# yupbank/tensorframes

Measured on AMD Instinct MI355X. Metric: rows/sec map_blocks MatMul on 10M-row DF at 1/2/4/8 MI355X, higher is better.
Workload: dtype fp32; 1 GPU; model=map_blocks relu(matmul(x[?,512], W[512,512])) float32, global_batch=10000000, seq_len=512, parallelism=dp1, partitions=4, rows=10000000

## Files before the change

### csrc/kernels/conv_wino.hip

```cpp
#include <algorithm>
#include <atomic>
#include <cstdlib>
#include <cstring>

#include "gemm_f32_core.h"

namespace tfa {
namespace k {

namespace {

typedef float f32x4 __attribute__((ext_vector_type(4)));
typedef float f32x16 __attribute__((ext_vector_type(16)));

struct WinoGeom {
  int H, W, C, OH, OW, pt, pl, TH, TW, OCP, KT;
  int64_t ntiles;
  int64_t img_floats;
  int64_t u_bytes;
  int dbg;
  int axis, D0, D1;
  FastDivU32 fD0, fD1;
  int KTC;
  FastDivU32 fKTC;
// ... 129 lines not shown
    }
    filt(1);
    filt(2);
#pragma unroll
    for (int m = 0; m < MT; ++m) {
      const f32x4 t3v = tr(inp(ra, 3, m), inp(rb, 3, m));
      av[3][m] = t1v[m] - t3v;
    }
    filt(3);
  };

  f32x16 acc[4][2];
  auto mfma_cols = [&](int j0, int j1, const f32x4 (&a)[4][MT], const f32x4 (&b)[4][NT]) __attribute__((always_inline)) {
#pragma unroll
    for (int j = j0; j < j1; ++j)
#pragma unroll
      for (int s = 0; s < 4; ++s)
#pragma unroll
        for (int m = 0; m < MT; ++m)
#pragma unroll
          for (int nh = 0; nh < NT; ++nh)
            acc[j][m * NT + nh] = __builtin_amdgcn_mfma_f32_32x32x2f32(a[j][m][s], b[j][nh][s], acc[j][m * NT + nh], 0, 0, 0);
  };
  f32x4 pa[4][MT], pb[4][NT];
  float* E = reinterpret_cast<float*>(smem + STAGE);

  int item = f32core::xcd_remap(blockIdx.x, G);
  if (item >= nwork) return;
  Item cur;
  setup(item, true, cur);
  issue(cur, 0);
  for (bool first = true;; first = false) {
#pragma unroll
    for (int j = 0; j < 4; ++j)
#pragma unroll
      for (int k2 = 0; k2 < 2; ++k2) acc[j][k2] = (f32x16){};
    for (int kt = 0; kt < KT; ++kt) {
      if (kt == 0 && !first) wwait_vm<NST>();
      else wwait_vm<0>();
      __builtin_amdgcn_s_barrier();
      if (kt + 1 < KT) issue(cur, kt + 1);
      if (kt > 0) mfma_cols(3, 4, pa, pb);
      read(kt);
      mfma_cols(0, 3, av, bv);
#pragma unroll
      for (int m = 0; m < MT; ++m) pa[3][m] = av[3][m];
#pragma unroll
      for (int nh = 0; nh < NT; ++nh) pb[3][nh] = bv[3][nh];
    }
    mfma_cols(3, 4, pa, pb);
    const int cq = lane % LPT, trr = lane / LPT;
    const int64_t col = cur.n0 + 4 * cq;
    const bool colok = col < g.N;
    float* cbase;
    int64_t cld;
    int cact;
    f32core::out_col(g, static_cast<float*>(g.C), colok ? col : 0, cbase, cld, cact);
    const float* bias = static_cast<const float*>(g.bias);
    const float4 bvv = (bias && colok) ? *reinterpret_cast<const float4*>(bias + col) : make_float4(0.f, 0.f, 0.f, 0.f);
    __syncthreads();
    const int next = item + G;
    const bool live = next < nwork;
    Item nx;
    setup(next, live, nx);
    issue(nx, 0);
    float4 pmax[NPASS];
#pragma unroll
    for (int px = 0; px < 2; ++px) {
#pragma unroll
      for (int m = 0; m < MT; ++m)
#pragma unroll
        for (int nh = 0; nh < NT; ++nh)
#pragma unroll
          for (int r = 0; r < 16; ++r) {
            const int k2 = m * NT + nh;
            const float mv = px == 0 ? (acc[0][k2][r] + acc[1][k2][r]) + acc[2][k2][r]
                                     : (acc[1][k2][r] - acc[2][k2][r]) - acc[3][k2][r];
            const int tile = (tp * MT + m) * TWV + (r & 3) + 8 * (r >> 2) + 4 * h;
            E[(xr * T + tile) * EP + 32 * nh + r32] = mv;
          }
      asm volatile("s_waitcnt lgkmcnt(0)" ::: "memory");
      __builtin_amdgcn_s_barrier();
#pragma unroll
      for (int ps = 0; ps < NPASS; ++ps) {
        const int tile = wave * (T / 8) + ps * TPP + trr;
        const int64_t t = cur.t0 + tile;
        const bool tl = t < q.ntiles;
        const uint32_t tc = tl ? (uint32_t)t : 0u, qa = fdiv(tc, q.fTW), tx = tc - qa * (uint32_t)q.TW;
        const uint32_t n = fdiv(qa, q.fTH), ty = qa - n * (uint32_t)q.TH;
        f32x4 e[4];
#pragma unroll
        for (int w = 0; w < 4; ++w) e[w] = *reinterpret_cast<const f32x4*>(&E[(w * T + tile) * EP + 4 * cq]);
        const f32x4 y0 = (e[0] + e[1]) + e[2];
        const f32x4 y1 = (e[1] - e[2]) - e[3];
        const int ow = 2 * (int)tx + px;
        float4 ov[2];
#pragma unroll
        for (int py = 0; py < 2; ++py) {
          const f32x4 v = py ? y1 : y0;
          ov[py].x = act3(v[0] + bvv.x, cact);
          ov[py].y = act3(v[1] + bvv.y, cact);
          ov[py].z = act3(v[2] + bvv.z, cact);
          ov[py].w = act3(v[3] + bvv.w, cact);
        }
        if constexpr (POOL) {
          const float4 m = make_float4(fmaxf(ov[0].x, ov[1].x), fmaxf(ov[0].y, ov[1].y), fmaxf(ov[0].z, ov[1].z),
                                       fmaxf(ov[0].w, ov[1].w));
          if (px == 0) {
            pmax[ps] = m;
          } else {
// ... 126 lines not shown
    av[7] = (d[7] - d[1]) + c21 * (d[3] - d[5]);
    const f32x4 e1 = (d[2] + d[6]) - c17 * d[4], o1 = (d[1] + d[5]) - c17 * d[3];
    av[1] = e1 + o1;
    av[2] = e1 - o1;
    const f32x4 e3 = (0.25f * d[2] + d[6]) - c5q * d[4], o3 = (0.5f * d[1] + 2.f * d[5]) - c5h * d[3];
    av[3] = e3 + o3;
    av[4] = e3 - o3;
    const f32x4 e5 = (4.f * d[2] + d[6]) - c5 * d[4], o5 = (2.f * d[1] + 0.5f * d[5]) - c5h * d[3];
    av[5] = e5 + o5;
    av[6] = e5 - o5;
  };

  f32x16 acc[8];
  auto mfma_pts = [&](int x0, int x1, const f32x4 (&a)[8], const f32x4 (&b)[8]) __attribute__((always_inline)) {
#pragma unroll
    for (int xi = x0; xi < x1; ++xi)
#pragma unroll
      for (int st = 0; st < 4; ++st) acc[xi] = __builtin_amdgcn_mfma_f32_32x32x2f32(a[xi][st], b[xi][st], acc[xi], 0, 0, 0);
  };
  f32x4 pa[8], pb[8];
  int item = f32core::xcd_remap(blockIdx.x, Gd);
  if (item >= nwork) return;
  Item cur;
  setup(item, true, cur);
  issue(cur, 0);
  for (bool first = true;; first = false) {
#pragma unroll
    for (int xi = 0; xi < 8; ++xi) acc[xi] = (f32x16){};
    if (S == 3 && KT > 1) issue(cur, 1);
    for (int kt = 0; kt < KT; ++kt) {
      const bool more = S == 3 && kt + 1 < KT;
      if (kt == 0 && !first) {
        if (more) wwait_vm<WFIRST>();
        else wwait_vm<WST>();
      } else if (more) {
        wwait_vm<G>();
      } else {
        wwait_vm<0>();
      }
      __builtin_amdgcn_s_barrier();
      if (kt + S - 1 < KT) issue(cur, kt + S - 1);
      if (kt > 0) mfma_pts(6, 8, pa, pb);
      read(kt);
      mfma_pts(0, 6, av, bv);
#pragma unroll
      for (int xi = 6; xi < 8; ++xi) {
        pa[xi] = av[xi];
        pb[xi] = bv[xi];
      }
    }
    mfma_pts(6, 8, pa, pb);
    const int64_t col = cur.n0 + nh * 32 + r32;
    const bool colok = col < g.N;
    float* cbase;
    int64_t cld;
    int cact;
    f32core::out_col(g, static_cast<float*>(g.C), colok ? col : 0, cbase, cld, cact);
    const float bias = (g.bias && colok) ? static_cast<const float*>(g.bias)[col] : 0.f;
    __syncthreads();
    const int next = item + Gd;
    const bool live = next < nwork;
    Item nx;
    setup(next, live, nx);
    issue(nx, 0);
#pragma unroll
    for (int r = 0; r < 16 && F45; ++r) {
      const float s12 = acc[1][r] - acc[2][r], s34 = acc[3][r] - acc[4][r], s56 = acc[5][r] - acc[6][r];
      const float a12 = acc[1][r] + acc[2][r], a34 = acc[3][r] + acc[4][r], a56 = acc[5][r] + acc[6][r];
      float y[4];
      y[0] = ((acc[0][r] + a12) + a34) + a56;
      y[1] = (s12 + 2.f * s34) + 0.5f * s56;
      y[2] = (a12 + 4.f * a34) + 0.25f * a56;
      y[3] = ((s12 + 8.f * s34) + 0.125f * s56) + acc[7][r];
      const int64_t t = cur.t0 + tq * 32 + (r & 3) + 8 * (r >> 2) + 4 * h;
      const bool tl = t < q.ntiles;
      uint32_t n;
      int oh, ow;
      tile_of(tl ? (uint32_t)t : 0u, n, oh, ow);
      const int64_t row0 = ((int64_t)n * q.OH + oh) * q.OW + ow;
      const bool ok0 = tl && colok && !(q.dbg & 4);
#pragma unroll
      for (int j = 0; j < 4; ++j) {
        const bool okj = ok0 && ow + j < q.OW;
        float* pj = okj ? cbase + (okj ? row0 + j : 0) * cld : reinterpret_cast<float*>(&kWinoTrash[lane]) + j;
        *pj = act3(y[j] + bias, cact);
      }
    }
#pragma unroll
    for (int r = 0; r < 16 && !F45; ++r) {
      const float y0 = ((((acc[0][r] + acc[1][r]) + (acc[2][r] + acc[3][r])) + (acc[4][r] + acc[5][r])) + acc[6][r]);
      const float y1 = (((acc[1][r] - acc[2][r]) + 2.f * (acc[3][r] - acc[4][r])) + 0.5f * (acc[5][r] - acc[6][r])) +
                       acc[7][r];
      const int64_t t = cur.t0 + tq * 32 + (r & 3) + 8 * (r >> 2) + 4 * h;
      const bool tl = t < q.ntiles;
      uint32_t n;
      int oh, ow;
      tile_of(tl ? (uint32_t)t : 0u, n, oh, ow);
      const int64_t row0 = ((int64_t)n * q.OH + oh) * q.OW + ow, step = dh ? q.OW : 1;
      const bool ok0 = tl && colok && !(q.dbg & 4);
      const bool ok1 = ok0 && (dh ? oh + 1 < q.OH : ow + 1 < q.OW);
      float* p0 = ok0 ? cbase + (ok0 ? row0 : 0) * cld : reinterpret_cast<float*>(&kWinoTrash[lane]);
      float* p1 = ok1 ? cbase + (ok1 ? row0 + step : 0) * cld : reinterpret_cast<float*>(&kWinoTrash[lane]) + 1;
      *p0 = act3(y0 + bias, cact);
      *p1 = act3(y1 + bias, cact);
    }
    if (!live) break;
    item = next;
    cur = nx;
  }
}
// ... 212 lines not shown
```

### csrc/kernels/gemm.hip

```cpp
#include <array>
#include <atomic>
#include <cmath>
#include <map>
#include <mutex>
#include <cstdlib>
#include <cstdio>
#include <cstring>
#include <string>
#include <type_traits>

#include "gemm_f32_core.h"
#include "gemm_g2_core.h"
#include "gemm_internal.h"
#include "hip_common.h"

namespace tfa {
namespace k {

namespace {

using namespace f32core;

__global__ __launch_bounds__(256) void splitk_reduce(const float* __restrict__ ws, GemmArgs g, int splits) {
  const int64_t M = g.M, N = g.N;
  const int64_t total = g.batch * M * N;
  const float* bias = static_cast<const float*>(g.bias);
  const int64_t stride = (int64_t)gridDim.x * blockDim.x;
  for (int64_t i = (int64_t)blockIdx.x * blockDim.x + threadIdx.x; i < total; i += stride) {
    float s = 0.f;
    for (int z = 0; z < splits; ++z) s += ws[z * total + i];
    const int64_t col = i % N;
    const int64_t row = (i / N) % M;
    const int64_t b = i / (M * N);
    if (bias) s += bias[col];
    float* cbase;
    int64_t cld;
    int cact;
    out_col(g, static_cast<float*>(g.C) + b * g.strideC, col, cbase, cld, cact);
    cbase[row * cld] = epi_apply(g.epi, act_apply(s, cact), row, col, N, b * M * N);
  }
}


constexpr int kFirstG2 = 22;
constexpr int kNumTiles = kFirstG2 + g2::kNumG2Tiles;
constexpr int kTiles[kNumTiles][2] = {{128, 128}, {128, 64}, {64, 128}, {64, 64}, {128, 32},
                                      {128, 96}, {128, 192}, {128, 160}, {64, 192}, {256, 128},
                                      {256, 64}, {256, 32}, {256, 96}, {256, 128}, {256, 96},
                                      {128, 128}, {128, 192}, {256, 64}, {128, 64}, {128, 256},
                                      {256, 256}, {256, 256},
                                      {256, 256}, {256, 192}, {256, 128}, {256, 64}, {128, 128}, {128, 64},
                                      {128, 192}, {256, 96}, {128, 160}, {192, 192}, {128, 224}};
static_assert(g2::kG2Tiles[0][0] == 256 && g2::kG2Tiles[0][1] == 256 && g2::kG2Tiles[5][1] == 64 &&
                  g2::kG2Tiles[6][1] == 192 && g2::kG2Tiles[7][1] == 96 && g2::kG2Tiles[8][1] == 160 &&
                  g2::kG2Tiles[9][0] == 192 && g2::kG2Tiles[10][1] == 224,
              "kTiles' g2 rows mirror kG2Tiles");

bool g2_ok(const GemmArgs& g, int al, bool vec) {
  static const bool off = [] {
    const char* e = std::getenv("TFA_GEMM_G2");
    return e && std::atoi(e) == 0;
  }();
  if (off || !vec || (al != A_KCONTIG && al != A_CONV)) return false;
  if (!g.tb && g.N % 4 != 0) return false;
  constexpr int64_t kMaxLd = (int64_t(1) << 32) / (256 * 4) - 64;
  if ((al == A_KCONTIG && g.lda > kMaxLd) || g.ldb > kMaxLd) return false;
  return g.K % 4 == 0;
}

int64_t tile_blocks(int c, int64_t M, int64_t N, int64_t batch) {
  return ((M + kTiles[c][0] - 1) / kTiles[c][0]) * ((N + kTiles[c][1] - 1) / kTiles[c][1]) * batch;
}

F32Plan plan_for(int cfg, int64_t M, int64_t N, int64_t K, int64_t batch) {
  F32Plan p{cfg, kTiles[cfg][0], kTiles[cfg][1], 1, K};
  const int64_t nb = tile_blocks(cfg, M, N, batch);
  if (nb < 256 && K >= 256) {
    int64_t s = std::min<int64_t>((512 + nb - 1) / nb, K / 128);
    s = std::max<int64_t>(1, std::min<int64_t>(s, 16));
    int64_t kps = ((K + s - 1) / s + kSplitAlign - 1) / kSplitAlign * kSplitAlign;
    p.splits = (int)((K + kps - 1) / kps);
    p.k_per_split = kps;
  }
  return p;
}

std::atomic<int>& forced_tile() {
  static std::atomic<int> v([] {
    const char* e = std::getenv("TFA_GEMM_TILE");
    const int t = e ? std::atoi(e) : -1;
    return t >= 0 && t < kNumTiles ? t : -1;
  }());
// ... 372 lines not shown
```

### csrc/kernels/gemm_f32_core.h

```cpp
#pragma once

#include <cstdint>
#include <cstdlib>
#include <type_traits>

#include "gemm_internal.h"
#include "hip_common.h"

namespace tfa {
namespace k {
namespace f32core {

enum ALoad { A_KCONTIG = 0, A_MCONTIG = 1, A_CONV = 2 };

struct ConvGeom {
  int H, W, C, KW, OH, OW, sh, sw, dh, dw, pt, pl;
  FastDivU32 fOW, fOH;
  bool fast = false;
};

constexpr int kBK = 16;
constexpr int kSplitAlign = 32;

struct F32Plan {
// ... 4 lines not shown
};

void launch_conv(const F32Plan& p, const GemmArgs& g, bool vec, const ConvGeom& cg, hipStream_t s);
void launch_kcontig_b(const F32Plan& p, const GemmArgs& g, bool vec, hipStream_t s);
void launch_kcontig_bt(const F32Plan& p, const GemmArgs& g, bool vec, hipStream_t s);
void launch_mcontig_b(const F32Plan& p, const GemmArgs& g, bool vec, hipStream_t s);
void launch_mcontig_bt(const F32Plan& p, const GemmArgs& g, bool vec, hipStream_t s);

namespace {

typedef float f32x16 __attribute__((ext_vector_type(16)));

__device__ __forceinline__ int xcd_remap(int b, int nwg) {
  const int q = nwg / 8, r = nwg % 8, x = b % 8;
  return (x < r ? x * (q + 1) : r * (q + 1) + (x - r) * q) + b / 8;
}



__device__ __attribute__((aligned(16))) float kZeroPage[4] = {0.f, 0.f, 0.f, 0.f};



__device__ __forceinline__ float4 ld4(const float* p, bool vec, bool ok0, bool ok1, bool ok2, bool ok3) {
  if (vec && ok3) return *reinterpret_cast<const float4*>(p);
  return make_float4(ok0 ? p[0] : 0.f, ok1 ? p[1] : 0.f, ok2 ? p[2] : 0.f, ok3 ? p[3] : 0.f);
}

template <bool VEC>
__device__ __forceinline__ float4 ld4_fast(const float* p) {
  if constexpr (VEC) return *reinterpret_cast<const float4*>(p);
  return make_float4(p[0], p[1], p[2], p[3]);
}

constexpr int kSchedMfma = 0x008, kSchedVmemRead = 0x020, kSchedDsRead = 0x100, kSchedDsWrite = 0x200;

template <int J, int END, int O1, int M1, int M2>
__device__ __forceinline__ void sched_ops() {
  if constexpr (J < END) {
    __builtin_amdgcn_sched_group_barrier(J < O1 ? M1 : M2, 1, 0);
    sched_ops<J + 1, END, O1, M1, M2>();
  }
}
template <int I, int NM, int O, int O1, int M1, int M2>
__device__ __forceinline__ void sched_interleave() {
  if constexpr (I < NM) {
    constexpr int lo = (I * O + NM - 1) / NM, hi = ((I + 1) * O + NM - 1) / NM;
    sched_ops<lo, hi, O1, M1, M2>();
    __builtin_amdgcn_sched_group_barrier(kSchedMfma, 1, 0);
    sched_interleave<I + 1, NM, O, O1, M1, M2>();
  }
}

__device__ __forceinline__ void out_col(const GemmArgs& g, float* Cb, int64_t col, float*& base, int64_t& ld,
                                        int& act) {
  if (g.seg.n == 0) {
    base = Cb + col;
    ld = g.ldc;
    act = g.act;
    return;
  }
  int s = 0;
#pragma unroll
  for (int q = 1; q < kMaxOutSegs; ++q)
    if (q < g.seg.n && col >= g.seg.begin[q]) s = q;
  base = static_cast<float*>(g.seg.ptr[s]) + (col - g.seg.begin[s]);
  ld = g.seg.ldc[s];
  act = g.seg.act[s];
}

template <int BM, int BN, int WM, int WN, int AL, bool TB, bool VEC, int BK>
__global__ __launch_bounds__(64 * WM * WN, (WM * WN == 16 ? 4 : (WM * WN == 8 ? 2 : (BM * BN > 128 * 192 ? 1 : 2))))
void gemm_f32_tile(GemmArgs g, int tiles_m, int tiles_n, ConvGeom cg, int64_t k_per_split, int flags) {
  constexpr int NT = 64 * WM * WN;
  constexpr int LDA = AL == A_MCONTIG ? BM + 4 : BM + 2;
  constexpr int LDB = TB ? BN + 2 : BN + 4;
  const int vepi = flags & 1;
  constexpr int TM = BM / WM / 32, TN = BN / WN / 32;
  static_assert((WM * WN == 4 || WM * WN == 8 || WM * WN == 16) && TM >= 1 && TN >= 1,
                "4, 8 or 16 waves, >= one 32x32 tile each");
  static_assert(BK % 8 == 0, "k is read in octets (k-step t: k = 8(t/4) + t%4 + 4 * half)");
  constexpr int KQ = BK / 4;
  constexpr int APIECES = BM * BK / 4, BPIECES = BN * BK / 4;
  constexpr int AP = (APIECES + NT - 1) / NT, BP = (BPIECES + NT - 1) / NT;
  constexpr int kStage = 32 * 32;
  constexpr int kMain = 2 * BK * (LDA + LDB), kEpi = (NT / 64) * kStage;
  __shared__ __attribute__((aligned(16))) float smem[kMain > kEpi ? kMain : kEpi];
  float(&As)[2][BK][LDA] = *reinterpret_cast<float(*)[2][BK][LDA]>(smem);
  float(&Bs)[2][BK][LDB] = *reinterpret_cast<float(*)[2][BK][LDB]>(smem + 2 * BK * LDA);

  const int tid = threadIdx.x;
  const int wave = tid >> 6, lane = tid & 63;
  const int wm = wave / WN, wn = wave % WN;
  const int nwg = tiles_m * tiles_n;
  const int wg = xcd_remap(blockIdx.x, nwg);
  const int64_t m0 = (int64_t)(wg / tiles_n) * BM;
  const int64_t n0 = (int64_t)(wg % tiles_n) * BN;
  const int64_t bz = blockIdx.y;
  const float* A = static_cast<const float*>(g.A) + bz * g.strideA;
  const float* B = static_cast<const float*>(g.B) + bz * g.strideB;
  const int64_t M = g.M, N = g.N, K = g.K;
  const int64_t kbeg = (int64_t)blockIdx.z * k_per_split;
  const int64_t kend = min(K, kbeg + k_per_split);
  constexpr bool v = VEC;

  int64_t cbase[AP];
  int cih[AP], ciw[AP];
  if (AL == A_CONV) {
#pragma unroll
    for (int p = 0; p < AP; ++p) {
      const int64_t m = m0 + (tid + NT * p) / KQ;
      cbase[p] = -1;
      cih[p] = ciw[p] = 0;
      if (m < M) {
        int64_t ow, oh, n;
        if (cg.fast) {
          const uint32_t m32 = (uint32_t)m, t = fdiv(m32, cg.fOW), q = fdiv(t, cg.fOH);
          ow = m32 - t * (uint32_t)cg.OW;
          oh = t - q * (uint32_t)cg.OH;
          n = q;
        } else {
// ... 169 lines not shown
  constexpr int S = BK / 2, NM = TM * TN, R = TM + TN;
  constexpr int L = (VEC ? 1 : 4) * (AP + BP);
  constexpr int W = AP * (AL == A_MCONTIG ? 1 : 4) + BP * (TB ? 4 : 1);
  auto mainloop = [&](auto chk) __attribute__((always_inline)) {
    if (ktiles > 0) {
      load(kbeg, chk);
      store(0);
    }
    __syncthreads();
    int cur = 0;
    auto tile = [&](int64_t knext, auto more) {
      constexpr bool NEXT = decltype(more)::value;
      float a[2][TM], b[2][TN];
      auto rd = [&](int buf, int t) {
        const int kr = 8 * (t >> 2) + (t & 3) + 4 * (lane >> 5);
#pragma unroll
        for (int i = 0; i < TM; ++i) a[buf][i] = As[cur][kr][wm * (BM / WM) + i * 32 + (lane & 31)];
#pragma unroll
        for (int j = 0; j < TN; ++j) b[buf][j] = Bs[cur][kr][wn * (BN / WN) + j * 32 + (lane & 31)];
      };
      rd(0, 0);
      __builtin_amdgcn_sched_group_barrier(kSchedDsRead, R, 0);
      if constexpr (NEXT) load(knext, chk);
#pragma unroll
      for (int kk = 0; kk < S; ++kk) {
        if (kk + 1 < S) rd((kk + 1) & 1, kk + 1);
        if (NEXT && kk == S - 1) store(cur ^ 1);
#pragma unroll
        for (int i = 0; i < TM; ++i)
#pragma unroll
          for (int j = 0; j < TN; ++j)
            acc[i][j] = __builtin_amdgcn_mfma_f32_32x32x2f32(a[kk & 1][i], b[kk & 1][j], acc[i][j], 0, 0, 0);
        if (kk == 0 && NEXT)
          sched_interleave<0, NM, L + R, L, kSchedVmemRead, kSchedDsRead>();
        else if (kk == S - 1 && NEXT)
          sched_interleave<0, NM, W, W, kSchedDsWrite, kSchedDsWrite>();
        else if (kk + 1 < S)
          sched_interleave<0, NM, R, R, kSchedDsRead, kSchedDsRead>();
        else
          __builtin_amdgcn_sched_group_barrier(kSchedMfma, NM, 0);
      }
      __syncthreads();
      cur ^= 1;
    };
    for (int kt = 0; kt + 1 < ktiles; ++kt) tile(kbeg + (int64_t)(kt + 1) * BK, std::true_type{});
    if (ktiles > 0) tile(0, std::false_type{});
  };
  const bool interior = m0 + BM <= M && n0 + BN <= N && (kend - kbeg) % BK == 0;
  if (interior)
    mainloop(std::false_type{});
  else
    mainloop(std::true_type{});

  float* ws = static_cast<float*>(g.workspace);
  const float* bias = static_cast<const float*>(g.bias);
  const bool heavy = !ws && !(g.act <= ACT_RELU6 && g.epi.n == 0);
  float* Cb = static_cast<float*>(g.C) + bz * g.strideC;
  if (vepi) {
    float* st = smem + wave * kStage;
    static_for<TN>([&](auto jc) __attribute__((always_inline)) {
      constexpr int j = decltype(jc)::value;
      static_for<TM>([&](auto ic) __attribute__((always_inline)) {
        constexpr int i = decltype(ic)::value;
        const f32x16 v = acc[i][j];
#pragma unroll
        for (int r = 0; r < 16; ++r) st[((r & 3) + 8 * (r >> 2) + 4 * (lane >> 5)) * 32 + (lane & 31)] = v[r];
        const int64_t col = n0 + wn * (BN / WN) + j * 32 + 4 * (lane & 7);
        if (col < N) {
          float* cbase;
          int64_t cld;
          int cact;
          out_col(g, Cb, col, cbase, cld, cact);
          float4 bv = make_float4(0.f, 0.f, 0.f, 0.f);
          if (bias) bv = make_float4(bias[col], bias[col + 1], bias[col + 2], bias[col + 3]);
#pragma unroll
          for (int q = 0; q < 4; ++q) {
            const int rr = 8 * q + (lane >> 3);
            const int64_t row = m0 + wm * (BM / WM) + i * 32 + rr;
            float4 o = *reinterpret_cast<const float4*>(&st[rr * 32 + 4 * (lane & 7)]);
            o.x = act_fast(o.x + bv.x, cact);
            o.y = act_fast(o.y + bv.y, cact);
            o.z = act_fast(o.z + bv.z, cact);
            o.w = act_fast(o.w + bv.w, cact);
            if (row < M) *reinterpret_cast<float4*>(cbase + row * cld) = o;
          }
        }
      });
    });
    return;
  }
  static_for<TN>([&](auto jc) __attribute__((always_inline)) {
    constexpr int j = decltype(jc)::value;
    const int64_t col = n0 + wn * (BN / WN) + j * 32 + (lane & 31);
    if (col >= N) return;
    const float bv = (!ws && bias) ? bias[col] : 0.f;
    float* cbase;
    int64_t cld;
    int cact;
    out_col(g, Cb, col, cbase, cld, cact);
    if (heavy) cact = ACT_NONE;
    static_for<TM>([&](auto ic) __attribute__((always_inline)) {
      constexpr int i = decltype(ic)::value;
      const f32x16 v = acc[i][j];
#pragma unroll
      for (int r = 0; r < 16; ++r) {
        const int64_t row = m0 + wm * (BM / WM) + i * 32 + (r & 3) + 8 * (r >> 2) + 4 * (lane >> 5);
        if (row >= M) continue;
        if (ws)
          ws[(((int64_t)blockIdx.z * gridDim.y + bz) * M + row) * N + col] = v[r];
        else
          cbase[row * cld] = act_fast(v[r] + bv, cact);
      }
    });
  });
  if (heavy) {
#pragma nounroll
    for (int e = 0; e < TN * TM * 16; ++e) {
      const int j = e / (TM * 16), i = (e / 16) % TM, r = e % 16;
      const int64_t col = n0 + wn * (BN / WN) + j * 32 + (lane & 31);
      const int64_t row = m0 + wm * (BM / WM) + i * 32 + (r & 3) + 8 * (r >> 2) + 4 * (lane >> 5);
      if (col >= N || row >= M) continue;
      float* cbase;
      int64_t cld;
      int cact;
      out_col(g, Cb, col, cbase, cld, cact);
      float* p = cbase + row * cld;
      *p = epi_apply(g.epi, act_apply(*p, cact), row, col, N, bz * M * N);
    }
  }
}

bool al16(const void* p) { return (reinterpret_cast<uintptr_t>(p) & 15) == 0; }

int vector_epilogue(const GemmArgs& g) {
  static const bool off = [] {
    const char* e = std::getenv("TFA_GEMM_VEC_EPILOGUE");
    return e && std::atoi(e) == 0;
  }();
  if (off || g.workspace || g.act > ACT_RELU6 || g.epi.n != 0 || g.N % 4 != 0) return 0;
  if (g.seg.n == 0) {
    if (!al16(g.C) || g.ldc % 4 != 0 || (g.batch > 1 && g.strideC % 4 != 0)) return 0;
  } else {
    for (int q = 0; q < g.seg.n; ++q)
      if (g.seg.begin[q] % 4 != 0 || g.seg.ldc[q] % 4 != 0 || !al16(g.seg.ptr[q]) || g.seg.act[q] > ACT_RELU6)
        return 0;
    if (g.seg.begin[g.seg.n] % 4 != 0) return 0;
  }
  return 1;
}

template <int AL, bool TB, bool VEC>
void launch_cfg(const F32Plan& p, const GemmArgs& g, const ConvGeom& cg, hipStream_t s) {
  const int vepi = p.splits == 1 ? vector_epilogue(g) : 0;
  const int64_t tm = (g.M + p.bm - 1) / p.bm, tn = (g.N + p.bn - 1) / p.bn;
  TFA_CHECK(tm * tn < (int64_t(1) << 31), "gemm: grid too large");
  TFA_CHECK(g.batch <= 65535 && p.splits <= 65535, "gemm: batch/splits too large");
  dim3 grid((unsigned)(tm * tn), (unsigned)g.batch, (unsigned)p.splits);
#define TFA_LAUNCH_TILE_BK(BM_, BN_, WM_, WN_, BK_)                                                         \
  hipLaunchKernelGGL((gemm_f32_tile<BM_, BN_, WM_, WN_, AL, TB, VEC, BK_>), grid, dim3(64 * WM_ * WN_), 0, s, g, \
                     (int)tm, (int)tn, cg, p.k_per_split, vepi)
#define TFA_LAUNCH_TILE(BM_, BN_, WM_, WN_) TFA_LAUNCH_TILE_BK(BM_, BN_, WM_, WN_, kBK)
  switch (p.cfg) {
    case 0: TFA_LAUNCH_TILE(128, 128, 2, 2); break;
    case 1: TFA_LAUNCH_TILE(128, 64, 2, 2); break;
    case 2: TFA_LAUNCH_TILE(64, 128, 2, 2); break;
    case 3: TFA_LAUNCH_TILE(64, 64, 2, 2); break;
    case 4: TFA_LAUNCH_TILE(128, 32, 4, 1); break;
    case 5: TFA_LAUNCH_TILE(128, 96, 4, 1); break;
    case 6: TFA_LAUNCH_TILE(128, 192, 2, 2); break;
    case 7: TFA_LAUNCH_TILE(128, 160, 4, 1); break;
    case 8: TFA_LAUNCH_TILE(64, 192, 2, 2); break;
    case 9: TFA_LAUNCH_TILE(256, 128, 2, 2); break;
    case 10: TFA_LAUNCH_TILE(256, 64, 4, 1); break;
    case 11: TFA_LAUNCH_TILE(256, 32, 4, 1); break;
    case 12: TFA_LAUNCH_TILE(256, 96, 4, 1); break;
    case 13: TFA_LAUNCH_TILE(256, 128, 4, 2); break;
    case 14: TFA_LAUNCH_TILE(256, 96, 8, 1); break;
    case 15: TFA_LAUNCH_TILE(128, 128, 2, 4); break;
    case 16: TFA_LAUNCH_TILE(128, 192, 4, 2); break;
    case 17: TFA_LAUNCH_TILE(256, 64, 8, 1); break;
    case 18: TFA_LAUNCH_TILE(128, 64, 4, 2); break;
    case 19: TFA_LAUNCH_TILE(128, 256, 4, 2); break;
// ... 12 lines not shown
```

### csrc/kernels/gemm_g2_core.h

```cpp
#pragma once

#include "gemm_f32_core.h"

namespace tfa {
namespace k {
namespace g2 {

using f32core::A_CONV;
using f32core::A_KCONTIG;
using f32core::ConvGeom;
using f32core::F32Plan;

enum BLoad { B_RC = 0, B_KC = 1 };
constexpr int A_CONV16 = 100;

void launch_kc(const F32Plan& p, const GemmArgs& g, hipStream_t s);
void launch_conv(const F32Plan& p, const GemmArgs& g, const ConvGeom& cg, hipStream_t s);

constexpr int kNumG2Tiles = 11;
constexpr int kG2Tiles[kNumG2Tiles][6] = {
    {256, 256, 2, 2, 4, 1}, {256, 192, 2, 2, 4, 1}, {256, 128, 2, 2, 3, 2}, {256, 64, 4, 1, 4, 2},
    {128, 128, 2, 2, 4, 2}, {128, 64, 2, 2, 5, 2},  {128, 192, 2, 2, 4, 2}, {256, 96, 4, 1, 3, 2},
    {128, 160, 4, 1, 4, 2}, {192, 192, 2, 2, 3, 2}, {128, 224, 4, 1, 3, 2}};

// ... 214 lines not shown
    for (int r = 0; r < TM + TN; ++r) read_frag(kt, j, r, f);
  };
  constexpr int KP = KQ / 2;
  constexpr int NM = 4 * TM * TN;
  constexpr int NR = TM + TN * (BL == B_KC ? 1 : 4);
  static_assert(KQ % 2 == 0, "whole k-quad pairs per stage");

  const int KT = kend > kbeg ? (int)((kend - kbeg + BK - 1) / BK) : 0;
#pragma unroll
  for (int s = 0; s < STAGES - 1; ++s) issue(s);
  wait_vm<G * (STAGES - 2)>();
  __builtin_amdgcn_s_barrier();
  Frag cur, nxt;
  read(0, 0, cur);
  auto stage = [&](int kt, auto do_issue, auto do_check) __attribute__((always_inline)) {
    constexpr bool ISSUE = decltype(do_issue)::value;
    if (ISSUE || kt + STAGES - 2 < KT) wait_vm<G * (STAGES - 3)>();
    else wait_vm<0>();
    __builtin_amdgcn_s_barrier();
    const int slot_next = (kt + STAGES - 1) % STAGES;
    static_for<KP>([&](auto jc) __attribute__((always_inline)) {
      constexpr int j = decltype(jc)::value;
      constexpr int p0 = 0, p1 = (ISSUE && j == 0) ? G : 0;
      constexpr int NP = p1 - p0;
      if constexpr (j + 1 < KP) read(kt, j + 1, nxt);
      else read(kt + 1, 0, nxt);
      static_for<NP>([&](auto pc) __attribute__((always_inline)) {
        issue_piece(slot_next, p0 + decltype(pc)::value, do_check);
      });
#pragma unroll
      for (int sk = 0; sk < 4; ++sk)
#pragma unroll
        for (int i = 0; i < TM; ++i)
#pragma unroll
          for (int jn = 0; jn < TN; ++jn)
            acc[i][jn] = __builtin_amdgcn_mfma_f32_32x32x2f32(cur.a[i][sk], cur.b[jn][sk], acc[i][jn], 0, 0, 0);
      static_for<NM>([&](auto xc) __attribute__((always_inline)) {
        constexpr int x = decltype(xc)::value;
        __builtin_amdgcn_sched_group_barrier(f32core::kSchedMfma, 1, 0);
        if constexpr (x < NP) __builtin_amdgcn_sched_group_barrier(f32core::kSchedVmemRead, 1, 0);
        else if constexpr (x < NP + NR) __builtin_amdgcn_sched_group_barrier(f32core::kSchedDsRead, 1, 0);
      });
      cur = nxt;
    });
  };
  int kt = 0;
  const int KTF = kend > kbeg ? (int)((kend - kbeg) / BK) : 0;
  if (m0 + BM <= M && n0 + BN <= N)
    for (; kt + STAGES - 1 < KTF; ++kt) stage(kt, std::true_type{}, std::false_type{});
  for (; kt + STAGES - 1 < KT; ++kt) stage(kt, std::true_type{}, std::true_type{});
  for (; kt < KT; ++kt) stage(kt, std::false_type{}, std::true_type{});
  __syncthreads();

  const int vepi = flags & 1;
  float* ws = static_cast<float*>(g.workspace);
  const float* bias = static_cast<const float*>(g.bias);
  const bool heavy = !ws && !(g.act <= ACT_RELU6 && g.epi.n == 0);
  float* Cb = static_cast<float*>(g.C) + bz * g.strideC;
  if (vepi) {
    float* stg = reinterpret_cast<float*>(smem) + wave * 1024;
    static_for<TN>([&](auto jc) __attribute__((always_inline)) {
      constexpr int j = decltype(jc)::value;
      static_for<TM>([&](auto ic) __attribute__((always_inline)) {
        constexpr int i = decltype(ic)::value;
        const f32x16 v = acc[i][j];
#pragma unroll
        for (int r = 0; r < 16; ++r) stg[((r & 3) + 8 * (r >> 2) + 4 * h) * 32 + r32] = v[r];
        const int64_t col = n0 + wn * (BN / WN) + j * 32 + 4 * (lane & 7);
        if (col < N) {
          float* cbase;
          int64_t cld;
          int cact;
          f32core::out_col(g, Cb, col, cbase, cld, cact);
          float4 bv = make_float4(0.f, 0.f, 0.f, 0.f);
          if (bias) bv = make_float4(bias[col], bias[col + 1], bias[col + 2], bias[col + 3]);
#pragma unroll
          for (int q = 0; q < 4; ++q) {
            const int rr = 8 * q + (lane >> 3);
            const int64_t row = m0 + wm * (BM / WM) + i * 32 + rr;
            float4 o = *reinterpret_cast<const float4*>(&stg[rr * 32 + 4 * (lane & 7)]);
            o.x = act_fast(o.x + bv.x, cact);
            o.y = act_fast(o.y + bv.y, cact);
            o.z = act_fast(o.z + bv.z, cact);
            o.w = act_fast(o.w + bv.w, cact);
            if (row < M) *reinterpret_cast<float4*>(cbase + row * cld) = o;
          }
        }
      });
    });
    return;
  }
  static_for<TN>([&](auto jc) __attribute__((always_inline)) {
    constexpr int j = decltype(jc)::value;
    const int64_t col = n0 + wn * (BN / WN) + j * 32 + r32;
    if (col >= N) return;
    const float bv = (!ws && bias) ? bias[col] : 0.f;
    float* cbase;
    int64_t cld;
    int cact;
    f32core::out_col(g, Cb, col, cbase, cld, cact);
    if (heavy) cact = ACT_NONE;
    static_for<TM>([&](auto ic) __attribute__((always_inline)) {
      constexpr int i = decltype(ic)::value;
      const f32x16 v = acc[i][j];
#pragma unroll
      for (int r = 0; r < 16; ++r) {
        const int64_t row = m0 + wm * (BM / WM) + i * 32 + (r & 3) + 8 * (r >> 2) + 4 * h;
        if (row >= M) continue;
        if (ws)
          ws[(((int64_t)blockIdx.z * gridDim.y + bz) * M + row) * N + col] = v[r];
        else
          cbase[row * cld] = act_fast(v[r] + bv, cact);
      }
    });
  });
  if (heavy) {
#pragma nounroll
    for (int e = 0; e < TN * TM * 16; ++e) {
      const int j = e / (TM * 16), i = (e / 16) % TM, r = e % 16;
      const int64_t col = n0 + wn * (BN / WN) + j * 32 + r32;
      const int64_t row = m0 + wm * (BM / WM) + i * 32 + (r & 3) + 8 * (r >> 2) + 4 * h;
      if (col >= N || row >= M) continue;
      float* cbase;
      int64_t cld;
      int cact;
      f32core::out_col(g, Cb, col, cbase, cld, cact);
      float* p = cbase + row * cld;
      *p = epi_apply(g.epi, act_apply(*p, cact), row, col, N, bz * M * N);
    }
  }
}

template <int AL, int BL>
void launch_cfg(const F32Plan& p, const GemmArgs& g, const ConvGeom& cg, hipStream_t s) {
  const int vepi = p.splits == 1 ? f32core::vector_epilogue(g) : 0;
  const int bm = kG2Tiles[p.cfg][0], bn = kG2Tiles[p.cfg][1];
  const int64_t tm = (g.M + bm - 1) / bm, tn = (g.N + bn - 1) / bn;
  TFA_CHECK(tm * tn < (int64_t(1) << 31), "gemm: grid too large");
  TFA_CHECK(g.batch <= 65535 && p.splits <= 65535, "gemm: batch/splits too large");
  dim3 grid((unsigned)(tm * tn), (unsigned)g.batch, (unsigned)p.splits);
#define TFA_G2(C_)                                                                                             \
  hipLaunchKernelGGL((g2_tile<kG2Tiles[C_][0], kG2Tiles[C_][1], kG2Tiles[C_][2], kG2Tiles[C_][3], kG2Tiles[C_][4], \
                              kG2Tiles[C_][5], AL, BL>),                                                         \
                     grid, dim3(64 * kG2Tiles[C_][2] * kG2Tiles[C_][3]), 0, s, g, (int)tm, (int)tn, cg,          \
                     p.k_per_split, vepi)
  switch (p.cfg) {
    case 0: TFA_G2(0); break;
    case 1: TFA_G2(1); break;
    case 2: TFA_G2(2); break;
    case 3: TFA_G2(3); break;
    case 4: TFA_G2(4); break;
    case 5: TFA_G2(5); break;
    case 6: TFA_G2(6); break;
    case 7: TFA_G2(7); break;
    case 8: TFA_G2(8); break;
    case 9: TFA_G2(9); break;
    default: TFA_G2(10); break;
  }
#undef TFA_G2
}

}
}
}
}
```

Before: 23.42 million rows/s.

## Unify GEMM epilogue with scalar-pinned output table and full-tile fast path

After: 23.35 million rows/s. About the same (-0.3%).

```diff
diff --git a/csrc/kernels/conv_wino.hip b/csrc/kernels/conv_wino.hip
--- a/csrc/kernels/conv_wino.hip
+++ b/csrc/kernels/conv_wino.hip
@@ -205,10 +205,11 @@
     const int cq = lane % LPT, trr = lane / LPT;
     const int64_t col = cur.n0 + 4 * cq;
     const bool colok = col < g.N;
-    float* cbase;
-    int64_t cld;
-    int cact;
-    f32core::out_col(g, static_cast<float*>(g.C), colok ? col : 0, cbase, cld, cact);
+    int64_t cend;
+    const f32core::OutDst od = f32core::out_at(f32core::out_tab(g, static_cast<float*>(g.C)), colok ? col : 0, cend);
+    float* cbase = od.base + (colok ? col : 0);
+    const int64_t cld = od.ld;
+    const int cact = od.act;
     const float* bias = static_cast<const float*>(g.bias);
     const float4 bvv = (bias && colok) ? *reinterpret_cast<const float4*>(bias + col) : make_float4(0.f, 0.f, 0.f, 0.f);
     __syncthreads();
@@ -441,10 +442,11 @@
     mfma_pts(6, 8, pa, pb);
     const int64_t col = cur.n0 + nh * 32 + r32;
     const bool colok = col < g.N;
-    float* cbase;
-    int64_t cld;
-    int cact;
-    f32core::out_col(g, static_cast<float*>(g.C), colok ? col : 0, cbase, cld, cact);
+    int64_t cend;
+    const f32core::OutDst od = f32core::out_at(f32core::out_tab(g, static_cast<float*>(g.C)), colok ? col : 0, cend);
+    float* cbase = od.base + (colok ? col : 0);
+    const int64_t cld = od.ld;
+    const int cact = od.act;
     const float bias = (g.bias && colok) ? static_cast<const float*>(g.bias)[col] : 0.f;
     __syncthreads();
     const int next = item + Gd;
diff --git a/csrc/kernels/gemm.hip b/csrc/kernels/gemm.hip
--- a/csrc/kernels/gemm.hip
+++ b/csrc/kernels/gemm.hip
@@ -26,6 +26,8 @@
   const int64_t total = g.batch * M * N;
   const float* bias = static_cast<const float*>(g.bias);
   const int64_t stride = (int64_t)gridDim.x * blockDim.x;
+  const OutTab t = out_tab(g, static_cast<float*>(g.C));
+  const int64_t sc = g.seg.n == 0 ? g.strideC : 0;
   for (int64_t i = (int64_t)blockIdx.x * blockDim.x + threadIdx.x; i < total; i += stride) {
     float s = 0.f;
     for (int z = 0; z < splits; ++z) s += ws[z * total + i];
@@ -33,11 +35,9 @@
     const int64_t row = (i / N) % M;
     const int64_t b = i / (M * N);
     if (bias) s += bias[col];
-    float* cbase;
-    int64_t cld;
-    int cact;
-    out_col(g, static_cast<float*>(g.C) + b * g.strideC, col, cbase, cld, cact);
-    cbase[row * cld] = epi_apply(g.epi, act_apply(s, cact), row, col, N, b * M * N);
+    int64_t end;
+    const OutDst d = out_at(t, col, end);
+    d.base[b * sc + row * d.ld + col] = epi_apply(g.epi, act_apply(s, d.act), row, col, N, b * M * N);
   }
 }
 
diff --git a/csrc/kernels/gemm_f32_core.h b/csrc/kernels/gemm_f32_core.h
--- a/csrc/kernels/gemm_f32_core.h
+++ b/csrc/kernels/gemm_f32_core.h
@@ -80,21 +80,233 @@
   }
 }
 
-__device__ __forceinline__ void out_col(const GemmArgs& g, float* Cb, int64_t col, float*& base, int64_t& ld,
-                                        int& act) {
-  if (g.seg.n == 0) {
-    base = Cb + col;
-    ld = g.ldc;
-    act = g.act;
+
+__device__ __forceinline__ int64_t wave_uniform(int64_t v) {
+  const uint32_t lo = (uint32_t)__builtin_amdgcn_readfirstlane((int)(uint32_t)v);
+  const uint32_t hi = (uint32_t)__builtin_amdgcn_readfirstlane((int)(uint32_t)((uint64_t)v >> 32));
+  return (int64_t)(((uint64_t)hi << 32) | lo);
+}
+__device__ __forceinline__ void pin_scalar(int& x) {
+  x = __builtin_amdgcn_readfirstlane(x);
+  asm volatile("" : "+s"(x));
+}
+__device__ __forceinline__ void pin_scalar(int64_t& x) {
+  x = wave_uniform(x);
+  asm volatile("" : "+s"(x));
+}
+__device__ __forceinline__ void pin_scalar(uint64_t& x) {
+  x = (uint64_t)wave_uniform((int64_t)x);
+  asm volatile("" : "+s"(x));
+}
+
+__device__ __forceinline__ float act_sel(float v, int act) {
+  const bool on = (act == ACT_RELU) | (act == ACT_RELU6);
+  const float r = (on & !(v > 0.f)) ? 0.f : v;
+  return ((act == ACT_RELU6) & (r > 6.f)) ? 6.f : r;
+}
+
+struct OutDst {
+  float* base;
+  int64_t ld;
+  int act;
+};
+
+struct OutTab {
+  int n;
+  int64_t begin[kMaxOutSegs + 1];
+  float* base[kMaxOutSegs];
+  int64_t ld[kMaxOutSegs];
+  int act[kMaxOutSegs];
+};
+
+__device__ __forceinline__ OutTab out_tab(const GemmArgs& g, float* Cb) {
+  OutTab t;
+  const bool one = g.seg.n == 0;
+  t.n = one ? 1 : g.seg.n;
+#pragma unroll
+  for (int q = 0; q < kMaxOutSegs; ++q) {
+    int64_t b = g.seg.begin[q], ld = g.seg.ldc[q];
+    uint64_t p = reinterpret_cast<uint64_t>(g.seg.ptr[q]);
+    int act = g.seg.act[q];
+    if (q == 0) {
+      b = one ? 0 : b;
+      ld = one ? g.ldc : ld;
+      p = one ? reinterpret_cast<uint64_t>(Cb) : p;
+      act = one ? g.act : act;
+    }
+    p -= (uint64_t)b * sizeof(float);
+    pin_scalar(b);
+    pin_scalar(ld);
+    pin_scalar(p);
+    pin_scalar(act);
+    t.begin[q] = b;
+    t.ld[q] = ld;
+    t.base[q] = (float*)(__attribute__((address_space(1))) float*)p;
+    t.act[q] = act;
+  }
+  int64_t e1 = one ? g.N : g.seg.begin[1], e = g.seg.begin[kMaxOutSegs];
+  pin_scalar(e1);
+  pin_scalar(e);
+  t.begin[1] = e1;
+  t.begin[kMaxOutSegs] = e;
+  return t;
+}
+
+__device__ __forceinline__ OutDst out_at(const OutTab& t, int64_t col, int64_t& end) {
+  OutDst d{t.base[0], t.ld[0], t.act[0]};
+  end = t.begin[1];
+#pragma unroll
+  for (int q = 1; q < kMaxOutSegs; ++q) {
+    const bool hit = (q < t.n) & (col >= t.begin[q]);
+    d.base = hit ? t.base[q] : d.base;
+    d.ld = hit ? t.ld[q] : d.ld;
+    d.act = hit ? t.act[q] : d.act;
+    end = hit ? t.begin[q + 1] : end;
+  }
+  return d;
+}
+
+template <bool CHECK, typename ActF>
+__device__ __forceinline__ void store_tile_vec(const f32x16& v, float* stg, int lane, float* p, int64_t ld,
+                                               const float4& bv, bool colok, int64_t nrows, ActF actf) {
+#pragma unroll
+  for (int r = 0; r < 16; ++r) stg[((r & 3) + 8 * (r >> 2) + 4 * (lane >> 5)) * 32 + (lane & 31)] = v[r];
+  const float* rd = stg + (lane >> 3) * 32 + 4 * (lane & 7);
+#pragma unroll
+  for (int q = 0; q < 4; ++q) {
+    float4 o = *reinterpret_cast<const float4*>(rd + 8 * q * 32);
+    o.x = actf(o.x + bv.x);
+    o.y = actf(o.y + bv.y);
+    o.z = actf(o.z + bv.z);
+    o.w = actf(o.w + bv.w);
+    if (!CHECK || (colok && 8 * q < nrows)) *reinterpret_cast<float4*>(p + 8 * q * ld) = o;
+  }
+}
+
+template <int TM, int TN>
+__device__ __forceinline__ void epilogue(const GemmArgs& g, f32x16 (&acc)[TM][TN], float* stg, int vepi, int lane,
+                                         int64_t rowb_, int64_t colb_, bool full, int64_t bz) {
+  const int64_t M = g.M, N = g.N;
+  const int64_t rowb = wave_uniform(rowb_), colb = wave_uniform(colb_);
+  const int h = lane >> 5, r32 = lane & 31;
+  if (float* ws = static_cast<float*>(g.workspace)) {
+    float* slab = ws + ((int64_t)blockIdx.z * gridDim.y + bz) * M * N;
+    static_for<TN>([&](auto jc) __attribute__((always_inline)) {
+      constexpr int j = decltype(jc)::value;
+      const int64_t col = colb + j * 32 + r32;
+      if (col >= N) return;
+      static_for<TM>([&](auto ic) __attribute__((always_inline)) {
+        constexpr int i = decltype(ic)::value;
+        const f32x16 v = acc[i][j];
+#pragma unroll
+        for (int r = 0; r < 16; ++r) {
+          const int64_t row = rowb + i * 32 + (r & 3) + 8 * (r >> 2) + 4 * h;
+          if (row < M) slab[row * N + col] = v[r];
+        }
+      });
+    });
     return;
   }
-  int s = 0;
-#pragma unroll
-  for (int q = 1; q < kMaxOutSegs; ++q)
-    if (q < g.seg.n && col >= g.seg.begin[q]) s = q;
-  base = static_cast<float*>(g.seg.ptr[s]) + (col - g.seg.begin[s]);
-  ld = g.seg.ldc[s];
-  act = g.seg.act[s];
+  const float* bias = static_cast<const float*>(g.bias);
+  float* Cb = static_cast<float*>(g.C) + bz * g.strideC;
+  if (vepi) {
+    const int c4 = 4 * (lane & 7), r8 = lane >> 3;
+    if (g.seg.n == 0 && full) {
+      const int64_t ld = g.ldc;
+      float* p0 = Cb + (rowb + r8) * ld + (colb + c4);
+      const float* bp = bias ? bias + (colb + c4) : nullptr;
+      auto run = [&](auto actc) __attribute__((always_inline)) {
+        constexpr int ACT = decltype(actc)::value;
+        static_for<TN>([&](auto jc) __attribute__((always_inline)) {
+          constexpr int j = decltype(jc)::value;
+          float4 bv = make_float4(0.f, 0.f, 0.f, 0.f);
+          if (bp) bv = make_float4(bp[j * 32], bp[j * 32 + 1], bp[j * 32 + 2], bp[j * 32 + 3]);
+          static_for<TM>([&](auto ic) __attribute__((always_inline)) {
+            constexpr int i = decltype(ic)::value;
+            store_tile_vec<false>(acc[i][j], stg, lane, p0 + (int64_t)(i * 32) * ld + j * 32, ld, bv, true, 0,
+                                  [](float x) { return act_fast(x, ACT); });
+          });
+        });
+      };
+      const int act = g.act;
+      if (act == ACT_RELU) run(std::integral_constant<int, ACT_RELU>{});
+      else if (act == ACT_RELU6) run(std::integral_constant<int, ACT_RELU6>{});
+      else run(std::integral_constant<int, ACT_NONE>{});
+      return;
+    }
+    const OutTab t = out_tab(g, Cb);
+    static_for<TN>([&](auto jc) __attribute__((always_inline)) {
+      constexpr int j = decltype(jc)::value;
+      const int64_t c0 = colb + j * 32;
+      if (c0 >= N) return;
+      const int64_t col = c0 + c4;
+      const bool colok = col < N;
+      float4 bv = make_float4(0.f, 0.f, 0.f, 0.f);
+      if (bias && colok) bv = make_float4(bias[col], bias[col + 1], bias[col + 2], bias[col + 3]);
+      int64_t end;
+      const OutDst d = out_at(t, c0, end);
+      auto tiles = [&](const OutDst& o) __attribute__((always_inline)) {
+        const int act = o.act;
+        static_for<TM>([&](auto ic) __attribute__((always_inline)) {
+          constexpr int i = decltype(ic)::value;
+          const int64_t row = rowb + i * 32 + r8;
+          store_tile_vec<true>(acc[i][j], stg, lane, o.base + row * o.ld + col, o.ld, bv, colok, M - row,
+                               [act](float x) { return act_sel(x, act); });
+        });
+      };
+      if ((c0 + 32 < N ? c0 + 32 : N) <= end) {
+        tiles(d);
+      } else {
+        int64_t e;
+        tiles(out_at(t, col, e));
+      }
+    });
+    return;
+  }
+  const bool heavy = !(g.act <= ACT_RELU6 && g.epi.n == 0);
+  const OutTab t = out_tab(g, Cb);
+  static_for<TN>([&](auto jc) __attribute__((always_inline)) {
+    constexpr int j = decltype(jc)::value;
+    const int64_t c0 = colb + j * 32;
+    if (c0 >= N) return;
+    const int64_t col = c0 + r32;
+    const bool colok = col < N;
+    const float bv = (bias && colok) ? bias[col] : 0.f;
+    int64_t end;
+    const OutDst d = out_at(t, c0, end);
+    auto tiles = [&](const OutDst& o) __attribute__((always_inline)) {
+      const int act = heavy ? (int)ACT_NONE : o.act;
+      float* pc = o.base + col;
+      static_for<TM>([&](auto ic) __attribute__((always_inline)) {
+        constexpr int i = decltype(ic)::value;
+        const f32x16 v = acc[i][j];
+#pragma unroll
+        for (int r = 0; r < 16; ++r) {
+          const int64_t row = rowb + i * 32 + (r & 3) + 8 * (r >> 2) + 4 * h;
+          if (colok && row < M) pc[row * o.ld] = act_sel(v[r] + bv, act);
+        }
+      });
+    };
+    if ((c0 + 32 < N ? c0 + 32 : N) <= end) {
+      tiles(d);
+    } else {
+      int64_t e;
+      tiles(out_at(t, col, e));
+    }
+  });
+  if (heavy) {
+#pragma nounroll
+    for (int e = 0; e < TN * TM * 16; ++e) {
+      const int j = e / (TM * 16), i = (e / 16) % TM, r = e % 16;
+      const int64_t col = colb + j * 32 + r32;
+      const int64_t row = rowb + i * 32 + (r & 3) + 8 * (r >> 2) + 4 * h;
+      if (col >= N || row >= M) continue;
+      int64_t end;
+      const OutDst d = out_at(t, col, end);
+      float* p = d.base + row * d.ld + col;
+      *p = epi_apply(g.epi, act_apply(*p, d.act), row, col, N, bz * M * N);
+    }
+  }
 }
 
 template <int BM, int BN, int WM, int WN, int AL, bool TB, bool VEC, int BK>
@@ -370,82 +582,8 @@
   else
     mainloop(std::true_type{});
 
-  float* ws = static_cast<float*>(g.workspace);
-  const float* bias = static_cast<const float*>(g.bias);
-  const bool heavy = !ws && !(g.act <= ACT_RELU6 && g.epi.n == 0);
-  float* Cb = static_cast<float*>(g.C) + bz * g.strideC;
-  if (vepi) {
-    float* st = smem + wave * kStage;
-    static_for<TN>([&](auto jc) __attribute__((always_inline)) {
-      constexpr int j = decltype(jc)::value;
-      static_for<TM>([&](auto ic) __attribute__((always_inline)) {
-        constexpr int i = decltype(ic)::value;
-        const f32x16 v = acc[i][j];
-#pragma unroll
-        for (int r = 0; r < 16; ++r) st[((r & 3) + 8 * (r >> 2) + 4 * (lane >> 5)) * 32 + (lane & 31)] = v[r];
-        const int64_t col = n0 + wn * (BN / WN) + j * 32 + 4 * (lane & 7);
-        if (col < N) {
-          float* cbase;
-          int64_t cld;
-          int cact;
-          out_col(g, Cb, col, cbase, cld, cact);
-          float4 bv = make_float4(0.f, 0.f, 0.f, 0.f);
-          if (bias) bv = make_float4(bias[col], bias[col + 1], bias[col + 2], bias[col + 3]);
-#pragma unroll
-          for (int q = 0; q < 4; ++q) {
-            const int rr = 8 * q + (lane >> 3);
-            const int64_t row = m0 + wm * (BM / WM) + i * 32 + rr;
-            float4 o = *reinterpret_cast<const float4*>(&st[rr * 32 + 4 * (lane & 7)]);
-            o.x = act_fast(o.x + bv.x, cact);
-            o.y = act_fast(o.y + bv.y, cact);
-            o.z = act_fast(o.z + bv.z, cact);
-            o.w = act_fast(o.w + bv.w, cact);
-            if (row < M) *reinterpret_cast<float4*>(cbase + row * cld) = o;
-          }
-        }
-      });
-    });
-    return;
-  }
-  static_for<TN>([&](auto jc) __attribute__((always_inline)) {
-    constexpr int j = decltype(jc)::value;
-    const int64_t col = n0 + wn * (BN / WN) + j * 32 + (lane & 31);
-    if (col >= N) return;
-    const float bv = (!ws && bias) ? bias[col] : 0.f;
-    float* cbase;
-    int64_t cld;
-    int cact;
-    out_col(g, Cb, col, cbase, cld, cact);
-    if (heavy) cact = ACT_NONE;
-    static_for<TM>([&](auto ic) __attribute__((always_inline)) {
-      constexpr int i = decltype(ic)::value;
-      const f32x16 v = acc[i][j];
-#pragma unroll
-      for (int r = 0; r < 16; ++r) {
-        const int64_t row = m0 + wm * (BM / WM) + i * 32 + (r & 3) + 8 * (r >> 2) + 4 * (lane >> 5);
-        if (row >= M) continue;
-        if (ws)
-          ws[(((int64_t)blockIdx.z * gridDim.y + bz) * M + row) * N + col] = v[r];
-        else
-          cbase[row * cld] = act_fast(v[r] + bv, cact);
-      }
-    });
-  });
-  if (heavy) {
-#pragma nounroll
-    for (int e = 0; e < TN * TM * 16; ++e) {
-      const int j = e / (TM * 16), i = (e / 16) % TM, r = e % 16;
-      const int64_t col = n0 + wn * (BN / WN) + j * 32 + (lane & 31);
-      const int64_t row = m0 + wm * (BM / WM) + i * 32 + (r & 3) + 8 * (r >> 2) + 4 * (lane >> 5);
-      if (col >= N || row >= M) continue;
-      float* cbase;
-      int64_t cld;
-      int cact;
-      out_col(g, Cb, col, cbase, cld, cact);
-      float* p = cbase + row * cld;
-      *p = epi_apply(g.epi, act_apply(*p, cact), row, col, N, bz * M * N);
-    }
-  }
+  epilogue<TM, TN>(g, acc, smem + wave * kStage, vepi, lane, m0 + wm * (BM / WM), n0 + wn * (BN / WN),
+                   m0 + BM <= M && n0 + BN <= N, bz);
 }
 
 bool al16(const void* p) { return (reinterpret_cast<uintptr_t>(p) & 15) == 0; }
diff --git a/csrc/kernels/gemm_g2_core.h b/csrc/kernels/gemm_g2_core.h
--- a/csrc/kernels/gemm_g2_core.h
+++ b/csrc/kernels/gemm_g2_core.h
@@ -290,83 +290,8 @@
   for (; kt < KT; ++kt) stage(kt, std::false_type{}, std::true_type{});
   __syncthreads();
 
-  const int vepi = flags & 1;
-  float* ws = static_cast<float*>(g.workspace);
-  const float* bias = static_cast<const float*>(g.bias);
-  const bool heavy = !ws && !(g.act <= ACT_RELU6 && g.epi.n == 0);
-  float* Cb = static_cast<float*>(g.C) + bz * g.strideC;
-  if (vepi) {
-    float* stg = reinterpret_cast<float*>(smem) + wave * 1024;
-    static_for<TN>([&](auto jc) __attribute__((always_inline)) {
-      constexpr int j = decltype(jc)::value;
-      static_for<TM>([&](auto ic) __attribute__((always_inline)) {
-        constexpr int i = decltype(ic)::value;
-        const f32x16 v = acc[i][j];
-#pragma unroll
-        for (int r = 0; r < 16; ++r) stg[((r & 3) + 8 * (r >> 2) + 4 * h) * 32 + r32] = v[r];
-        const int64_t col = n0 + wn * (BN / WN) + j * 32 + 4 * (lane & 7);
-        if (col < N) {
-          float* cbase;
-          int64_t cld;
-          int cact;
-          f32core::out_col(g, Cb, col, cbase, cld, cact);
-          float4 bv = make_float4(0.f, 0.f, 0.f, 0.f);
-          if (bias) bv = make_float4(bias[col], bias[col + 1], bias[col + 2], bias[col + 3]);
-#pragma unroll
-          for (int q = 0; q < 4; ++q) {
-            const int rr = 8 * q + (lane >> 3);
-            const int64_t row = m0 + wm * (BM / WM) + i * 32 + rr;
-            float4 o = *reinterpret_cast<const float4*>(&stg[rr * 32 + 4 * (lane & 7)]);
-            o.x = act_fast(o.x + bv.x, cact);
-            o.y = act_fast(o.y + bv.y, cact);
-            o.z = act_fast(o.z + bv.z, cact);
-            o.w = act_fast(o.w + bv.w, cact);
-            if (row < M) *reinterpret_cast<float4*>(cbase + row * cld) = o;
-          }
-        }
-      });
-    });
-    return;
-  }
-  static_for<TN>([&](auto jc) __attribute__((always_inline)) {
-    constexpr int j = decltype(jc)::value;
-    const int64_t col = n0 + wn * (BN / WN) + j * 32 + r32;
-    if (col >= N) return;
-    const float bv = (!ws && bias) ? bias[col] : 0.f;
-    float* cbase;
-    int64_t cld;
-    int cact;
-    f32core::out_col(g, Cb, col, cbase, cld, cact);
-    if (heavy) cact = ACT_NONE;
-    static_for<TM>([&](auto ic) __attribute__((always_inline)) {
-      constexpr int i = decltype(ic)::value;
-      const f32x16 v = acc[i][j];
-#pragma unroll
-      for (int r = 0; r < 16; ++r) {
-        const int64_t row = m0 + wm * (BM / WM) + i * 32 + (r & 3) + 8 * (r >> 2) + 4 * h;
-        if (row >= M) continue;
-        if (ws)
-          ws[(((int64_t)blockIdx.z * gridDim.y + bz) * M + row) * N + col] = v[r];
-        else
-          cbase[row * cld] = act_fast(v[r] + bv, cact);
-      }
-    });
-  });
-  if (heavy) {
-#pragma nounroll
-    for (int e = 0; e < TN * TM * 16; ++e) {
-      const int j = e / (TM * 16), i = (e / 16) % TM, r = e % 16;
-      const int64_t col = n0 + wn * (BN / WN) + j * 32 + r32;
-      const int64_t row = m0 + wm * (BM / WM) + i * 32 + (r & 3) + 8 * (r >> 2) + 4 * h;
-      if (col >= N || row >= M) continue;
-      float* cbase;
-      int64_t cld;
-      int cact;
-      f32core::out_col(g, Cb, col, cbase, cld, cact);
-      float* p = cbase + row * cld;
-      *p = epi_apply(g.epi, act_apply(*p, cact), row, col, N, bz * M * N);
-    }
-  }
+  f32core::epilogue<TM, TN>(g, acc, reinterpret_cast<float*>(smem) + wave * 1024, flags & 1, lane,
+                            m0 + wm * (BM / WM), n0 + wn * (BN / WN), m0 + BM <= M && n0 + BN <= N, bz);
 }
 
 template <int AL, int BL>
diff --git a/profiles/epilogue/count_epilogue.py b/profiles/epilogue/count_epilogue.py
--- /dev/null
+++ b/profiles/epilogue/count_epilogue.py
@@ -0,0 +1,28 @@
+import re
+import sys
+from collections import Counter
+
+lines = open(sys.argv[1]).read().split("\n")
+pat = sys.argv[2]
+start = next(i for i, l in enumerate(lines) if re.match(r"^_Z\w*:", l) and pat in l)
+end = next(i for i in range(start, len(lines)) if lines[i].startswith(".Lfunc_end"))
+ins = [l.strip() for l in lines[start:end] if l.startswith("\t") and not l.strip().startswith((".", ";"))]
+ops = [x.split()[0] for x in ins]
+last_mfma = max(i for i, x in enumerate(ops) if x.startswith("v_mfma"))
+epi, c = ins[last_mfma + 1:], Counter(ops[last_mfma + 1:])
+
+
+def grp(pred):
+    return sum(v for k, v in c.items() if pred(k))
+
+
+print("kernel:", lines[start][:100])
+print("instructions:", len(ins), " after the last MFMA:", len(epi))
+print("ds_write*:", grp(lambda k: k.startswith("ds_write")), " ds_read*:", grp(lambda k: k.startswith("ds_read")))
+print("global_store*:", grp(lambda k: k.startswith("global_store")), " flat_store*:",
+      grp(lambda k: k.startswith("flat_store")), " global_load*:", grp(lambda k: k.startswith("global_load")),
+      " flat_load*:", grp(lambda k: k.startswith("flat_load")))
+print("branches:", grp(lambda k: k.startswith("s_cbranch") or k == "s_branch"),
+      " exec save/restore:", grp(lambda k: "saveexec" in k))
+print("v_cndmask:", grp(lambda k: k.startswith("v_cndmask")), " s_load*:", grp(lambda k: k.startswith("s_load")))
+print("s_waitcnt vmcnt(0):", sum(1 for x in epi if x.startswith("s_waitcnt") and "vmcnt(0)" in x))
diff --git a/profiles/epilogue/fit.py b/profiles/epilogue/fit.py
--- /dev/null
+++ b/profiles/epilogue/fit.py
@@ -0,0 +1,18 @@
+import json
+import sys
+
+import numpy as np
+
+best = {}
+for line in open(sys.argv[1]):
+    if not line.startswith("{"):
+        continue
+    d = json.loads(line)
+    k = int(d["dims"][2])
+    best[k] = min(best.get(k, 1e9), d["ms"])
+ks = sorted(best)
+A = np.array([[1.0, k] for k in ks])
+y = np.array([best[k] for k in ks])
+(a, b), *_ = np.linalg.lstsq(A, y, rcond=None)
+print("fit: min ms per K", {k: round(best[k], 4) for k in ks})
+print(f"fit: ms = a + b*K, a = {a:.4f} ms, b = {b * 1e3:.4f} us/k, a / ms(K=512) = {100 * a / best[512]:.2f} %")
diff --git a/profiles/epilogue/pmc_sum.py b/profiles/epilogue/pmc_sum.py
--- /dev/null
+++ b/profiles/epilogue/pmc_sum.py
@@ -0,0 +1,15 @@
+import csv
+import sys
+from collections import defaultdict
+
+rows = list(csv.DictReader(open(sys.argv[1])))
+by = defaultdict(lambda: defaultdict(list))
+for r in rows:
+    name = r.get("Kernel_Name", "")
+    if "g2_tile" not in name and "gemm_f32_tile" not in name:
+        continue
+    by[name[:90]][r["Counter_Name"]].append(float(r["Counter_Value"]))
+for name, cs in by.items():
+    print(name)
+    for c, v in sorted(cs.items()):
+        print(f"  {c:24s} n={len(v):3d} last={v[-1]:.4g} min={min(v):.4g}")
```
